# yuansliu/minicom

Measured on AMD Instinct MI355X. Metric: Mreads/s (sketch+index+overlap) on 150bp reads, 1/2/4/8 GPU; bit-exact decompress, higher is better.
Workload: dtype u64

## Files before the change

minicom_amd/csrc/api.hip:

```cpp
#include "mcom_dev.hpp"
#include "../../include/mcom_test.h"
#include <stdarg.h>
#include <stdlib.h>
#include <cxxabi.h>
#include <stdio.h>
#include <string.h>

int mcom_fail(mcom_ctx *ctx, int code, const char *fmt, ...)
{
	char buf[512];
	va_list ap;
	va_start(ap, fmt);
	vsnprintf(buf, sizeof buf, fmt, ap);
	va_end(ap);
	if (ctx) { ctx->err = buf; ctx->pin_wait.clear(); ctx->pin_off = 0; }
	return code;
}

#define MCOM_PIN_BYTES 4096
hipError_t mcom_d2h_async(mcom_ctx *ctx, void *dst, const void *src, size_t bytes)
{
	for (uint32_t q = 0; q < 8; ++q) {
		const mcom_ctx::ScanTotal &t = ctx->scan_last[(ctx->scan_last_at + 7u - q) % 8u];
		if (t.last && t.last == src && t.bytes == bytes && t.gen == ctx->launch_gen) { mcom_ctx::PinWait w{dst, 0, bytes}; w.from = ctx->scan_tot + t.slot; ctx->pin_wait.push_back(w); return hipSuccess; }
// ... 287 lines not shown
{
	if (!ctx || !name) return 0;
	if (!strcmp(name, "sort_overflow_segments")) return ctx->sort_overflow_segments;
	if (!strcmp(name, "sketch_strings")) return ctx->sketch_strings;
	return 0;
}
extern "C" int mcom_set_segment_capacity(mcom_ctx *ctx, uint32_t records)
{
	if (!ctx || records > 4096) return MCOM_E_ARG;
	ctx->seg_cap = records;
	return MCOM_OK;
}
extern "C" int mcom_set_consensus_capacity(mcom_ctx *ctx, uint32_t members)
{
	if (!ctx) return MCOM_E_ARG;
	ctx->bs_cap = members;
	return MCOM_OK;
}
extern "C" int mcom_set_sketch_kernel(mcom_ctx *ctx, int wave_per_string)
{
	if (!ctx) return MCOM_E_ARG;
	ctx->sketch_wave_only = wave_per_string == 1;
	ctx->sketch_ring64 = wave_per_string == 2;
	ctx->sketch_ring32_only = wave_per_string == 3;
	ctx->sketch_lane_always = wave_per_string >= 2;
	return MCOM_OK;
}
extern "C" int mcom_set_sketch_prefix_bits(mcom_ctx *ctx, int bits)
{
	if (!ctx || bits < 1 || bits > 30) return MCOM_E_ARG;
	ctx->sketch_prefix_bits = bits;
	return MCOM_OK;
}
extern "C" int mcom_set_claim_route(mcom_ctx *ctx, int route)
{
	if (!ctx || route < 0 || route > 3) return MCOM_E_ARG;
	ctx->claim_route = route;
	return MCOM_OK;
}
extern "C" int mcom_claim_fallbacks(const mcom_ctx *ctx) { return ctx ? (int)ctx->claim_fallbacks : 0; }
extern "C" int mcom_set_screen_route(mcom_ctx *ctx, int route)
{
	if (!ctx || route < 0 || route > 2) return MCOM_E_ARG;
	ctx->screen_route = route;
	return MCOM_OK;
}
extern "C" int mcom_screen_fallbacks(const mcom_ctx *ctx) { return ctx ? (int)ctx->screen_fallbacks : 0; }
extern "C" int mcom_set_lookup_route(mcom_ctx *ctx, int route)
{
	if (!ctx || route < 0 || route > 1) return MCOM_E_ARG;
	ctx->lookup_route = route;
	return MCOM_OK;
}
extern "C" int mcom_set_index_capacity(mcom_ctx *ctx, int entries)
{
	if (!ctx) return MCOM_E_ARG;
	ctx->cix_cap_set = entries >= 0; ctx->cix_cap = entries >= 0 ? (uint32_t)entries : 0u;
	return MCOM_OK;
}
```

minicom_amd/csrc/consensus_bs.hip:

```cpp
#include "mcom_dev.hpp"

#define BS_K 5
#define BS_NMAX 31u
#define BS_KM 7
#define BS_EVEN 0x5555555555555555ull

namespace {
template <int K> struct BsCnt { uint64_t p[K], q[K]; };

template <int K> __device__ __forceinline__ void bs_add(BsCnt<K> &c, uint64_t P, uint64_t Q)
{
#pragma unroll
	for (int b = 0; b < K; ++b) { uint64_t t = c.p[b] & P; c.p[b] ^= P; P = t; t = c.q[b] & Q; c.q[b] ^= Q; Q = t; }
}
template <int K> __device__ __forceinline__ void bs_sub(BsCnt<K> &c, uint64_t P, uint64_t Q)
{
#pragma unroll
	for (int b = 0; b < K; ++b) { uint64_t t = ~c.p[b] & P; c.p[b] ^= P; P = t; t = ~c.q[b] & Q; c.q[b] ^= Q; Q = t; }
}
template <int K> __device__ __forceinline__ void bs_best(const BsCnt<K> &c, uint64_t &lo, uint64_t &hi, uint64_t &nz)
{
	uint64_t best[K], cand[K];
#pragma unroll
	for (int b = 0; b < K; ++b) best[b] = c.p[b] & BS_EVEN;
	lo = 0; hi = 0;
	auto challenge = [&](int code) {
		uint64_t gt = 0, eq = BS_EVEN;
#pragma unroll
		for (int b = K - 1; b >= 0; --b) { gt |= eq & cand[b] & ~best[b]; eq &= ~(cand[b] ^ best[b]); }
#pragma unroll
		for (int b = 0; b < K; ++b) best[b] = (cand[b] & gt) | (best[b] & ~gt);
		lo = (code & 1) ? (lo | gt) : (lo & ~gt);
		hi = (code & 2) ? (hi | gt) : (hi & ~gt);
	};
#pragma unroll
	for (int b = 0; b < K; ++b) cand[b] = (c.p[b] >> 1) & BS_EVEN;
	challenge(1);
#pragma unroll
	for (int b = 0; b < K; ++b) cand[b] = c.q[b] & BS_EVEN;
	challenge(2);
#pragma unroll
	for (int b = 0; b < K; ++b) cand[b] = (c.q[b] >> 1) & BS_EVEN;
	challenge(3);
	nz = 0;
#pragma unroll
	for (int b = 0; b < K; ++b) nz |= best[b];
}
__device__ __forceinline__ uint64_t bs_rev(uint64_t x)
{
	x = __brevll(x);
	return ((x >> 1) & BS_EVEN) | ((x & BS_EVEN) << 1);
}
__device__ __forceinline__ uint64_t bs_span(int a, int b)
{
	if (b <= a) return 0;
	const uint64_t mb = b >= 32 ? ~0ull : ((1ull << (2 * b)) - 1), ma = (1ull << (2 * a)) - 1;
	return BS_EVEN & mb & ~ma;
}

#define BS_ORDER_GRID 1024
__global__ __launch_bounds__(256) void k_bs_sizes(const uint32_t *__restrict__ goff, uint32_t ng, uint32_t *__restrict__ bins)
{
	__shared__ uint32_t h[33];
	if (threadIdx.x < 33) h[threadIdx.x] = 0;
	__syncthreads();
	const uint32_t chunks = (ng + 255u) / 256u, per = (chunks + gridDim.x - 1) / gridDim.x;
	const uint32_t c0 = blockIdx.x * per, c1 = c0 + per < chunks ? c0 + per : chunks;
	for (uint32_t c = c0; c < c1; ++c) {
		const uint32_t g = c * 256u + threadIdx.x;
		if (g < ng) { const uint32_t n = goff[g + 1] - goff[g]; atomicAdd(&h[n < 32u ? n : 32u], 1u); }
	}
	__syncthreads();
	if (threadIdx.x < 33 && h[threadIdx.x]) atomicAdd(&bins[threadIdx.x], h[threadIdx.x]);
}
__global__ __launch_bounds__(256) void k_bs_order(const uint32_t *__restrict__ goff, uint32_t ng, const uint32_t *__restrict__ bins,
                                                  uint32_t *__restrict__ cursor, uint32_t *__restrict__ perm)
{
	__shared__ uint32_t h[33], base[33];
	if (threadIdx.x < 33) h[threadIdx.x] = 0;
	__syncthreads();
	const uint32_t chunks = (ng + 255u) / 256u, per = (chunks + gridDim.x - 1) / gridDim.x;
	const uint32_t c0 = blockIdx.x * per, c1 = c0 + per < chunks ? c0 + per : chunks;
	for (uint32_t c = c0; c < c1; ++c) {
		const uint32_t g = c * 256u + threadIdx.x;
		if (g < ng) { const uint32_t n = goff[g + 1] - goff[g]; atomicAdd(&h[n < 32u ? n : 32u], 1u); }
	}
	__syncthreads();
	if (threadIdx.x < 33) {
		const uint32_t b = threadIdx.x;
		uint32_t start = 0;
		if (b == 32) { for (uint32_t q = 0; q < 32; ++q) start += bins[q]; }
		else for (uint32_t q = b + 1; q < 32; ++q) start += bins[q];
		base[b] = start + (h[b] ? atomicAdd(&cursor[b], h[b]) : 0u);
		h[b] = 0;
	}
	__syncthreads();
	for (uint32_t c = c0; c < c1; ++c) {
		const uint32_t g = c * 256u + threadIdx.x;
		if (g < ng) { const uint32_t n = goff[g + 1] - goff[g], bin = n < 32u ? n : 32u; perm[base[bin] + atomicAdd(&h[bin], 1u)] = g; }
	}
}

__global__ __launch_bounds__(64) void k_group_consensus_bs(const uint64_t *__restrict__ packed, int W, uint64_t *__restrict__ members,
                                                           const uint32_t *__restrict__ goff, const uint32_t *__restrict__ perm, uint32_t nsmall,
                                                           int L, int k_orig, int e, int LG, int GPW,
                                                           uint8_t *__restrict__ keep, uint32_t *__restrict__ nkept,
                                                           uint16_t *__restrict__ svout, uint16_t *__restrict__ reflen,
                                                           uint8_t *__restrict__ refs, int ref_stride)
{
	__shared__ uint32_t S[2][64];
	__shared__ uint32_t M[64];
	__shared__ uint64_t CODE[64 + 64];
	const int lane = threadIdx.x;
	const int gs = lane / LG, u = lane - gs * LG;
	const uint32_t idx = blockIdx.x * (uint32_t)GPW + (uint32_t)gs;
	const bool valid = gs < GPW && idx < nsmall;
	const int TL = 2 * L;
	const uint32_t g = valid ? perm[idx] : 0u;
	const uint32_t m0 = valid ? goff[g] : 0u;
	const uint32_t n = valid ? goff[g + 1] - m0 : 0u;
	uint32_t nmax = n;
#pragma unroll
	for (int d = 32; d >= 1; d >>= 1) { const uint32_t o = (uint32_t)__shfl_xor((int)nmax, d, 64); nmax = o > nmax ? o : nmax; }
	S[0][lane] = 0; S[1][lane] = 0;
	const int col0 = 32 * u;
	int pos0 = 0;
	if (n) { const uint64_t y = members[m0]; int pos = (int)((uint32_t)y >> 1); if (y & 1) pos = L - pos + k_orig - 2; pos0 = pos; }
	struct Fetch { uint64_t y, wa, wb; int off, s0, sh; bool covered; };
	auto fetch_y = [&](uint32_t i) -> uint64_t { return i < n ? members[m0 + i] : 0ull; };
	auto fetch_rows = [&](uint32_t i, uint64_t y) -> Fetch {
		Fetch f; f.y = y;
		const uint32_t dir = (uint32_t)(y & 1);
		int pos = (int)((uint32_t)y >> 1);
		if (dir) pos = L - pos + k_orig - 2;
		f.off = pos0 - pos;
		f.s0 = col0 - f.off;
		f.covered = i < n && f.s0 < L && f.s0 + 32 > 0;
		const int t0 = dir ? L - 32 - f.s0 : f.s0;
		const int wj = t0 >> 5;
		f.sh = 2 * (t0 & 31);
		const uint64_t *row = packed + (size_t)(y >> 32) * W;
		f.wa = (f.covered && wj >= 0 && wj < W) ? row[wj] : 0ull;
		f.wb = (f.covered && f.sh && wj + 1 >= 0 && wj + 1 < W) ? row[wj + 1] : 0ull;
		return f;
	};
	auto finish = [&](const Fetch &f, uint64_t &x, uint64_t &cov) {
		x = f.sh ? (f.wa >> f.sh) | (f.wb << (64 - f.sh)) : f.wa;
		if (f.y & 1) x = ~bs_rev(x);
		cov = f.covered ? bs_span(f.s0 < 0 ? -f.s0 : 0, L - f.s0 < 32 ? L - f.s0 : 32) : 0ull;
	};
	auto planes = [&](uint64_t x, uint64_t cov, uint64_t &P, uint64_t &Q) {
		const uint64_t lo = x & BS_EVEN, hi = (x >> 1) & BS_EVEN;
		const uint64_t nh = cov & ~hi, hh = cov & hi;
		P = (nh & ~lo) | ((nh & lo) << 1);
		Q = (hh & ~lo) | ((hh & lo) << 1);
	};
	BsCnt<BS_K> c;
#pragma unroll
	for (int b = 0; b < BS_K; ++b) { c.p[b] = 0; c.q[b] = 0; }
	{
		uint64_t yn = fetch_y(0);
		Fetch cur = fetch_rows(0, yn);
		yn = fetch_y(1);
		for (uint32_t i = 0; i < nmax; ++i) {
			const Fetch nxt = fetch_rows(i + 1, yn);
			yn = fetch_y(i + 2);
			uint64_t x, cov, P, Q;
			finish(cur, x, cov);
			planes(x, cov, P, Q);
			bs_add(c, P, Q);
			cur = nxt;
		}
	}
	uint64_t rlo, rhi, nz;
	bs_best(c, rlo, rhi, nz);
	if (u == 0) M[gs] = (uint32_t)TL;
	__syncthreads();
	{
		const uint64_t empty = ~nz & BS_EVEN;
		if (valid && empty) { const int cnd = col0 + (__ffsll((unsigned long long)empty) - 1) / 2; if (cnd < TL) atomicMin(&M[gs], (uint32_t)cnd); }
	}
	__syncthreads();
	const int ref_len = (int)M[gs];
	const uint64_t inref = bs_span(0, ref_len - col0 < 0 ? 0 : (ref_len - col0 > 32 ? 32 : ref_len - col0));
	uint32_t nk = 0; int rend = 0;
	uint64_t yn = fetch_y(0);
	Fetch cur = fetch_rows(0, yn);
	yn = fetch_y(1);
	for (uint32_t i = 0; i < nmax; ++i) {
		const Fetch nxt = fetch_rows(i + 1, yn);
		yn = fetch_y(i + 2);
		uint64_t x, cov, P, Q;
		finish(cur, x, cov);
		const uint64_t y = cur.y; const int off = cur.off;
		const uint64_t lo = x & BS_EVEN, hi = (x >> 1) & BS_EVEN;
		const uint64_t mis = cov & (((lo ^ rlo) | (hi ^ rhi)) | ~inref);
		const uint32_t slot = i & 1u;
		if (mis) atomicAdd(&S[slot][gs], (uint32_t)__popcll(mis));
		__builtin_amdgcn_wave_barrier();
		const uint32_t dif = ((volatile uint32_t*)S[slot])[gs];
		__builtin_amdgcn_wave_barrier();
		if (u == 0) ((volatile uint32_t*)S[slot ^ 1u])[gs] = 0;
		const bool act = i < n;
		const bool kp = (int)dif <= e;
		if (act && kp) { ++nk; if (off + L > rend) rend = off + L; }
		if (__ballot(act && !kp)) {
			planes(x, (act && !kp) ? cov : 0ull, P, Q);
			bs_sub(c, P, Q);
		}
		if (act && u == 0) { keep[m0 + i] = kp ? 1 : 0; members[m0 + i] = (y >> 32 << 32) | ((uint64_t)off << 1) | (y & 1); }
		cur = nxt;
	}
	bs_best(c, rlo, rhi, nz);
	__syncthreads();
	if (u == 0) M[gs] = (uint32_t)ref_len;
	CODE[gs * (LG + 1) + u] = rlo | (rhi << 1);
	if (u == 0) CODE[gs * (LG + 1) + LG] = 0;
	__syncthreads();
	{
		const uint64_t first = nz & inref;
		if (valid && nk && first) atomicMin(&M[gs], (uint32_t)(col0 + (__ffsll((unsigned long long)first) - 1) / 2));
	}
	__syncthreads();
	const int sv = nk ? (int)M[gs] : 0;
	if (valid && nk) {
		uint8_t *out = refs + (size_t)g * ref_stride;
		const uint32_t *w32 = (const uint32_t*)&CODE[gs * (LG + 1)];
		const int n_out = rend - sv;
		for (int d = u; 4 * d < n_out; d += LG) {
			const int bit = 2 * (sv + 4 * d), wi = bit >> 5, sh = bit & 31;
			uint32_t v = w32[wi] >> sh;
			if (sh > 24) v |= w32[wi + 1] << (32 - sh);
			uint32_t ascii = 0;
#pragma unroll
			for (int r = 0; r < 4; ++r) ascii |= ((0x54474341u >> (8 * ((v >> (2 * r)) & 3u))) & 0xFFu) << (8 * r);
			if (4 * d + 4 <= n_out) *(uint32_t*)(out + 4 * d) = ascii;
			else for (int r = 0; 4 * d + r < n_out; ++r) out[4 * d + r] = (uint8_t)(ascii >> (8 * r));
		}
	}
	if (valid && u == 0) { nkept[g] = nk; svout[g] = (uint16_t)sv; reflen[g] = (uint16_t)(nk ? rend - sv : 0); }
}

__global__ __launch_bounds__(64) void k_merge_consensus_bs(const uint64_t *__restrict__ packed, int W, const uint64_t *__restrict__ members,
                                                           const uint64_t *__restrict__ joff, const uint64_t *__restrict__ roff,
                                                           const uint32_t *__restrict__ ujob, const uint32_t *__restrict__ uoff, uint32_t n_units, int L,
                                                           uint8_t *__restrict__ refs, const uint32_t *__restrict__ reg_lo, const uint32_t *__restrict__ reg_hi,
                                                           const uint32_t *__restrict__ toff, unsigned int *__restrict__ tflag, uint32_t *__restrict__ tlist,
                                                           unsigned int *__restrict__ tcount, uint32_t depth_cap)
{
	const uint32_t q = blockIdx.x * 64u + threadIdx.x;
	const bool valid = q < n_units;
	const uint32_t j = valid ? ujob[q] : 0u;
	long lo = 0, hi = 0, c0 = 0;
	uint64_t m0 = 0, m1 = 0;
	if (valid) {
		hi = reg_hi ? (long)reg_hi[j] : (long)(roff[j + 1] - roff[j]);
		lo = reg_lo ? (long)reg_lo[j] : 0;
		c0 = lo + 32l * (long)(q - uoff[j]);
		m0 = joff[j]; m1 = joff[j + 1];
	}
	const long ce = c0 + 32 < hi ? c0 + 32 : hi;
	uint64_t a = m0, b = m1;
	while (a < b) { const uint64_t mid = (a + b) >> 1; if ((long)((uint32_t)members[mid] >> 1) + L <= c0) a = mid + 1; else b = mid; }
	BsCnt<BS_KM> c;
// ... 30 lines not shown
				const int sh = 2 * (t0 & 31);
				uint64_t x = sh ? (wa >> sh) | (wb << (64 - sh)) : wa;
				if (dir) x = ~bs_rev(x);
				const int e0 = L - s0 < (int)(ce - c0) ? L - s0 : (int)(ce - c0);
				const uint64_t cov = bs_span(s0 < 0 ? -s0 : 0, e0);
				const uint64_t xl = x & BS_EVEN, xh = (x >> 1) & BS_EVEN;
				const uint64_t nh = cov & ~xh, hh = cov & xh;
				bs_add(c, (nh & ~xl) | ((nh & xl) << 1), (hh & ~xl) | ((hh & xl) << 1));
				++n;
			}
			++i;
			y = y1; wa = wa1; wb = wb1; y1 = y2;
		}
	}
	if (!valid) return;
	if (over) {
		const uint32_t t = toff[j] + (uint32_t)((c0 - lo) >> 9);
		if (atomicExch(&tflag[t], 1u) == 0u) tlist[atomicAdd(tcount, 1u)] = t;
		return;
	}
	uint64_t rlo, rhi, nz;
	bs_best(c, rlo, rhi, nz);
	const uint64_t code = rlo | (rhi << 1);
	uint8_t *out = refs + roff[j] + c0;
	const int cnt = (int)(ce - c0);
#pragma unroll
	for (int d = 0; d < 8; ++d) {
		if (4 * d >= cnt) break;
		const uint32_t v = (uint32_t)(code >> (8 * d)) & 0xFFu;
		uint32_t ascii = 0;
#pragma unroll
		for (int r = 0; r < 4; ++r) ascii |= ((0x54474341u >> (8 * ((v >> (2 * r)) & 3u))) & 0xFFu) << (8 * r);
		if (4 * d + 4 <= cnt) __builtin_memcpy(out + 4 * d, &ascii, 4);
		else for (int r = 0; 4 * d + r < cnt; ++r) out[4 * d + r] = (uint8_t)(ascii >> (8 * r));
	}
}
}

int mcom_group_consensus_small(mcom_ctx *ctx, const uint64_t *d_packed, uint64_t *d_members, const uint32_t *d_group_off, uint32_t n_groups,
                               int L, int k_orig, int e, uint8_t *d_keep, uint32_t *d_nkept, uint16_t *d_sv, uint16_t *d_reflen, uint8_t *d_refs,
                               int ref_stride, uint32_t **d_perm_out, uint32_t *n_small)
{
	*d_perm_out = nullptr; *n_small = 0;
	uint32_t *perm = nullptr;
	if (mcom_dmalloc(&perm, ((size_t)n_groups + 128) * 4) != hipSuccess) return mcom_fail(ctx, MCOM_E_NOMEM, "group order");
	uint32_t *bins = (uint32_t*)mcom_zeroed(ctx, perm + n_groups, 80 * 4), *cursor = bins ? bins + 40 : nullptr;
	hipError_t er = bins ? hipSuccess : hipErrorUnknown;
	const unsigned blocks = std::min<unsigned>((n_groups + 255) / 256, BS_ORDER_GRID);
	if (er == hipSuccess) {
		MCOM_LAUNCH(k_bs_sizes, dim3(blocks), dim3(256), 0, ctx->stream, d_group_off, n_groups, bins);
		MCOM_LAUNCH(k_bs_order, dim3(blocks), dim3(256), 0, ctx->stream, d_group_off, n_groups, bins, cursor, perm);
		er = hipGetLastError();
	}
	uint32_t nbig = 0;
	if (er == hipSuccess) er = mcom_d2h_async(ctx, &nbig, bins + 32, 4);
	if (er == hipSuccess) er = mcom_stream_sync(ctx);
	if (er != hipSuccess) { mcom_dfree(perm); return mcom_fail(ctx, MCOM_E_HIP, "group order: %s", hipGetErrorString(er)); }
	const uint32_t nsmall = n_groups - nbig;
	const int LG = (2 * L + 31) / 32, GPW = 64 / LG;
	if (nsmall) {
		McomProfScope ps_(ctx, PROF_CONSENSUS);
		MCOM_LAUNCH(k_group_consensus_bs, dim3((nsmall + GPW - 1) / GPW), dim3(64), 0, ctx->stream, d_packed, mcom_words_per_read(L), d_members, d_group_off, perm,
		                   nsmall, L, k_orig, e, LG, GPW, d_keep, d_nkept, d_sv, d_reflen, d_refs, ref_stride);
	}
	er = hipGetLastError();
	if (er != hipSuccess) { mcom_dfree(perm); return mcom_fail(ctx, MCOM_E_HIP, "group consensus: %s", hipGetErrorString(er)); }
	*d_perm_out = perm; *n_small = nsmall;
	return MCOM_OK;
}

int mcom_merge_consensus_units(mcom_ctx *ctx, const uint64_t *d_packed, const uint64_t *d_members, const uint64_t *d_job_off, const uint64_t *d_ref_off,
                               const uint32_t *d_ujob, const uint32_t *d_uoff, uint32_t n_units, int L, uint8_t *d_refs,
                               const uint32_t *d_reg_lo, const uint32_t *d_reg_hi, const uint32_t *d_toff, uint32_t n_tiles,
                               unsigned int *d_tflag, uint32_t *d_tlist, uint32_t *h_nlist)
{
	*h_nlist = 0;
	if (n_units == 0) return MCOM_OK;
	unsigned int *tcount = d_tflag + n_tiles;
	MCOM_HIP(ctx, hipMemsetAsync(d_tflag, 0, ((size_t)n_tiles + 1) * 4, ctx->stream));
	{
		McomProfScope ps_(ctx, PROF_CONSENSUS);
		MCOM_LAUNCH(k_merge_consensus_bs, dim3((n_units + 63) / 64), dim3(64), 0, ctx->stream, d_packed, mcom_words_per_read(L), d_members, d_job_off, d_ref_off,
		                   d_ujob, d_uoff, n_units, L, d_refs, d_reg_lo, d_reg_hi, d_toff, d_tflag, d_tlist, tcount,
		                   ctx->bs_cap && ctx->bs_cap < (1u << BS_KM) ? ctx->bs_cap : (1u << BS_KM) - 1u);
	}
	MCOM_LAUNCH_CHECK(ctx);
	MCOM_HIP(ctx, mcom_d2h_async(ctx, h_nlist, tcount, 4));
	MCOM_HIP(ctx, mcom_stream_sync(ctx));
	return MCOM_OK;
}
```

minicom_amd/csrc/mcom_dev.hpp:

```cpp
#pragma once
#include <hip/hip_runtime.h>
#include <stdint.h>
#include <stddef.h>
#include <map>
#include <string>
#include <vector>
#include "../../include/mcom.h"

enum McomProfId { PROF_CLASSIFY_PACK = 0, PROF_SKETCH_READS, PROF_RADIX_PASS, PROF_SKETCH_CONTIGS, PROF_FIND_NEXT,
                  PROF_DICT_BUILD, PROF_REALIGN_WINDOWS, PROF_CONSENSUS, PROF_CINDEX_BUILD, PROF_REALIGN_READS, PROF_COUNT };
struct McomProfSpan { int id; hipEvent_t a, b; };

struct mcom_ctx {
	int device;
	hipStream_t stream;
	std::string err;
	void *ws; size_t ws_bytes;
	int n_cu;
	bool prof_on = false;
	std::vector<McomProfSpan> prof_open;
	double prof_ms[PROF_COUNT] = {0};
	uint64_t prof_calls[PROF_COUNT] = {0};
	int prof_cur = PROF_COUNT;
	std::map<std::pair<int, const void *>, uint64_t> prof_kernels;
	uint32_t seg_cap = 0; uint64_t sort_overflow_segments = 0;
	uint64_t sketch_strings = 0;
	bool cix_cap_set = false; uint32_t cix_cap = 0;
	uint32_t bs_cap = 0;
	bool sketch_wave_only = false;
	bool sketch_lane_always = false;
	bool sketch_ring64 = false, sketch_ring32_only = false; int sketch_prefix_bits = 14;
	unsigned long long *scan_parts = nullptr; uint32_t scan_epoch = 0; volatile unsigned int *poison = nullptr; unsigned int *d_poison = nullptr;
	enum { SCAN_TOTALS = 64 };
	unsigned long long *scan_tot = nullptr, *d_scan_tot = nullptr;
	struct ScanTotal { const void *last; uint32_t bytes, slot, gen; } scan_last[8] = {}; uint32_t scan_last_at = 0, launch_gen = 1;
	int claim_route = 0; uint64_t claim_fallbacks = 0;
	unsigned int *screen_flag = nullptr;
	std::vector<void*> free_later;
	int screen_route = 0; uint64_t screen_fallbacks = 0;
	int lookup_route = 0;
	int verify_hash_bits = 64;
	struct ScreenArgs { const uint64_t *sgbits; size_t n_sg; int L, ininumdict, maxsearch, n_shares, share; } screen_args = {};
	enum { ZPOOL_BYTES = 64 * 1024 };
	unsigned char *zpool = nullptr; size_t zpool_used = 0; int zpool_half = 0;
	struct PinWait { void *dst; size_t off, bytes; const void *from = nullptr; };
	unsigned char *pin = nullptr; size_t pin_off = 0;
	std::vector<PinWait> pin_wait;
};

hipEvent_t mcom_prof_event_get();
void mcom_prof_event_put(hipEvent_t e);
struct McomProfScope {
	mcom_ctx *ctx; int idx;
	McomProfScope(mcom_ctx *c, int id) : ctx(c), idx(-1) {
		if (!c->prof_on) return;
		McomProfSpan s; s.id = id;
		if (!(s.a = mcom_prof_event_get())) return;
		if (!(s.b = mcom_prof_event_get())) { mcom_prof_event_put(s.a); return; }
		(void)hipEventRecord(s.a, c->stream);
		c->prof_open.push_back(s); idx = (int)c->prof_open.size() - 1;
		prev = c->prof_cur; c->prof_cur = id;
	}
	~McomProfScope() { if (idx >= 0) { (void)hipEventRecord(ctx->prof_open[idx].b, ctx->stream); ctx->prof_cur = prev; } }
	int prev = PROF_COUNT;
};
#define MCOM_LAUNCH(kernel, grid, block, lds, stream, ...) do { \
	++ctx->launch_gen; \
	if (ctx->prof_on) ++ctx->prof_kernels[std::make_pair(ctx->prof_cur, (const void*)&kernel)]; \
	hipLaunchKernelGGL(kernel, grid, block, lds, stream, __VA_ARGS__); } while (0)

int mcom_fail(mcom_ctx *ctx, int code, const char *fmt, ...);
hipError_t mcom_d2h_async(mcom_ctx *ctx, void *dst, const void *src, size_t bytes);
hipError_t mcom_stream_sync(mcom_ctx *ctx);
hipError_t mcom_stream_sync_poison(mcom_ctx *ctx, bool *poisoned);
int mcom_ws_reserve(mcom_ctx *ctx, size_t bytes);
void *mcom_zeroed(mcom_ctx *ctx, void *fallback, size_t bytes);
void mcom_ring_flush_slot(mcom_ctx *ctx, uint32_t slot);
unsigned long long *mcom_ring_slot(mcom_ctx *ctx, uint32_t *slot);
void mcom_ring_register(mcom_ctx *ctx, const void *d_result, uint32_t bytes, uint32_t slot);
hipError_t mcom_dmalloc(void **out, size_t bytes);
void mcom_dfree(void *p);
void mcom_dfree_later(mcom_ctx *ctx, void *p);
template <class T> static inline hipError_t mcom_dmalloc(T **out, size_t bytes) { return mcom_dmalloc((void**)out, bytes); }

int mcom_scan_u32(mcom_ctx *ctx, const uint32_t *in, uint32_t *out, size_t n, uint32_t *scratch);
size_t mcom_scan_scratch_elems(size_t n);
int mcom_scan_prepare(mcom_ctx *ctx);
size_t mcom_sort_ws_bytes(size_t n);
int mcom_sort_by_x(mcom_ctx *ctx, mcom_mm128 *d_a, size_t n, int bits, void *ws);
int mcom_sort_by_low_bits(mcom_ctx *ctx, mcom_mm128 *d_a, size_t n, int bits, void *ws);
int mcom_sort_by_low_bits_into_ws(mcom_ctx *ctx, const mcom_mm128 *d_src, mcom_mm128 *d_a, size_t n, int bits, void *ws, mcom_mm128 **d_sorted);
#define MCOM_GROUP_TILE 1280
#define MCOM_GROUP_SCRATCH(n) (4 * ((size_t)(n) / MCOM_GROUP_TILE + 1) + 16)
// ... 133 lines not shown
```

minicom_amd/hip.py:

```python
from __future__ import annotations

import ctypes as C
import os
import re

import numpy as np

HERE = os.path.dirname(os.path.abspath(__file__))
MM_DTYPE = np.dtype([("x", "<u8"), ("y", "<u8")])


class McomError(RuntimeError):
    pass


class DecodeSrc(C.Structure):
    _fields_ = [("d_text", C.c_void_p), ("text_bytes", C.c_uint64), ("d_line_start", C.c_void_p), ("verbatim", C.c_int),
                ("d_ref", C.c_void_p), ("ref_bytes", C.c_uint64), ("ref_const", C.c_int),
                ("d_cid", C.c_void_p), ("d_pos", C.c_void_p), ("d_coff", C.c_void_p), ("n_contigs", C.c_uint64),
                ("d_dir", C.c_void_p), ("dir_bytes", C.c_uint64)]


DECODE_F_BOUNDS, DECODE_F_LINE, DECODE_F_DUP, DECODE_F_DEST = 1, 2, 4, 8

# ... 131 lines not shown
    L.mcom_decode_pe_dest.restype = i32; L.mcom_decode_pe_dest.argtypes = [vp, vp, u64, u64, u64, vp, u64, u64, u64, vp, C.POINTER(u64), vp]
    L.mcom_decode_check_lines.restype = i32; L.mcom_decode_check_lines.argtypes = [vp, vp, u64, vp, u64, i32, i32, vp]
    L.mcom_decode_reads.restype = i32; L.mcom_decode_reads.argtypes = [vp, C.POINTER(DecodeSrc), u64, i32, vp, u64, vp, u64, vp, vp]
    L.mcom_verify_room.restype = u64; L.mcom_verify_room.argtypes = [u64, u64]
    L.mcom_verify_ordered.restype = i32; L.mcom_verify_ordered.argtypes = [vp, C.POINTER(VerifyTable), C.POINTER(VerifyTable), i32, C.POINTER(VerifyReport)]
    L.mcom_verify_multiset.restype = i32; L.mcom_verify_multiset.argtypes = [vp, C.POINTER(VerifyTable), C.POINTER(VerifyTable), i32, C.POINTER(VerifyReport)]
    L.mcom_set_verify_hash_bits.restype = i32; L.mcom_set_verify_hash_bits.argtypes = [vp, i32]
    L.mcom_rans_bound.restype = u64; L.mcom_rans_bound.argtypes = [u64]
    L.mcom_rans_encode.restype = i32; L.mcom_rans_encode.argtypes = [vp, vp, u64, vp, u64, C.POINTER(u64), i32]
    L.mcom_rans_decode.restype = i32; L.mcom_rans_decode.argtypes = [vp, vp, u64, vp, u64, C.POINTER(u64)]
    L.mcom_fastq_quality_rows.restype = i32; L.mcom_fastq_quality_rows.argtypes = [vp, vp, u64, vp, u64, u64, C.c_uint32, vp, u64, vp]
    L.mcom_fastq_emit.restype = i32; L.mcom_fastq_emit.argtypes = [vp, vp, u64, vp, u64, u64, u64, C.c_uint32, vp, C.POINTER(u64)]
    L.mcom_qual_bound.restype = u64; L.mcom_qual_bound.argtypes = [u64, C.c_uint32]
    L.mcom_qual_encode.restype = i32; L.mcom_qual_encode.argtypes = [vp, vp, u64, C.c_uint32, u64, vp, u64, C.POINTER(u64), i32]
    L.mcom_qual_gather_rows.restype = i32; L.mcom_qual_gather_rows.argtypes = [vp, vp, u64, C.c_uint32, u64, vp, u64, vp, u64, vp]
    L.mcom_dump_read_order.restype = i32; L.mcom_dump_read_order.argtypes = [vp, vp, u64, vp, u64, C.c_uint32, vp, C.POINTER(u64)]
    L.mcom_verify_multiset_parts.restype = i32; L.mcom_verify_multiset_parts.argtypes = [vp, C.POINTER(VerifyParts), C.POINTER(VerifyParts), i32, C.POINTER(VerifyReport)]
    L.mcom_qual_info.restype = i32; L.mcom_qual_info.argtypes = [vp, u64, C.POINTER(u64), C.POINTER(C.c_uint32)]
    L.mcom_qual_decode.restype = i32; L.mcom_qual_decode.argtypes = [vp, vp, u64, vp, u64, u64, C.POINTER(u64), C.POINTER(C.c_uint32)]
    L.mcom_name_bound.restype = u64; L.mcom_name_bound.argtypes = [u64]
    L.mcom_name_encode.restype = i32; L.mcom_name_encode.argtypes = [vp, vp, u64, u64, vp, u64, C.POINTER(u64), C.POINTER(u64)]
    L.mcom_name_info.restype = i32; L.mcom_name_info.argtypes = [vp, u64, C.POINTER(u64), C.POINTER(u64)]
    L.mcom_name_decode.restype = i32; L.mcom_name_decode.argtypes = [vp, vp, u64, vp, u64, C.POINTER(u64), C.POINTER(u64), vp]
    L.mcom_name_text_offsets.restype = i32; L.mcom_name_text_offsets.argtypes = [vp, vp, u64, u64, vp]
    L.mcom_name_compare.restype = i32; L.mcom_name_compare.argtypes = [vp, vp, vp, u64, vp, vp, u64, u64, C.POINTER(u64), C.POINTER(u64)]
    L.mcom_fastq_name_text.restype = i32; L.mcom_fastq_name_text.argtypes = [vp, vp, u64, vp, u64, u64, vp, u64, C.POINTER(u64), vp, vp]
    L.mcom_fastq_emit_named.restype = i32; L.mcom_fastq_emit_named.argtypes = [vp, vp, u64, vp, u64, vp, u64, vp, u64, C.c_uint32, vp, C.POINTER(u64)]
    L.mcom_bwt_bound.restype = u64; L.mcom_bwt_bound.argtypes = [u64]
    L.mcom_bwt_encode.restype = i32; L.mcom_bwt_encode.argtypes = [vp, vp, u64, vp, u64, C.POINTER(u64)]
    L.mcom_bwt_decode.restype = i32; L.mcom_bwt_decode.argtypes = [vp, vp, u64, vp, u64, C.POINTER(u64)]
    L.mcom_synth_reads.restype = i32
    L.mcom_synth_reads.argtypes = [vp, u64, u64, i32, i32, C.c_double, u64, u64, vp, sz]
    L.mcom_synth_reads_genome.restype = i32
    L.mcom_synth_reads_genome.argtypes = [vp, u64, u64, i32, i32, C.c_double, i32, u64, u64, vp, sz]
    _lib = L
    return L


def words_per_read(L: int) -> int:
    return (2 * L + 63) // 64


def _torch():
    import torch
    return torch


class Context:

    def __init__(self, device: int = 0, stream=None):
        torch = _torch()
        if not torch.cuda.is_available():
            raise McomError("no GPU visible: the minicom_amd product path has no CPU fallback")
        self.lib = load_library()
        self.device = torch.device("cuda", device)
        torch.cuda.set_device(self.device)
        self._stream = stream if stream is not None else torch.cuda.current_stream(self.device)
        h = C.c_void_p()
        rc = self.lib.mcom_create(C.byref(h), device, C.c_void_p(self._stream.cuda_stream))
        if rc:
            raise McomError(f"mcom_create failed ({rc})")
        self._h = h

    def close(self):
        if getattr(self, "_h", None):
            self.lib.mcom_destroy(self._h)
            self._h = None

    def __del__(self):
        try:
            self.close()
        except Exception:
            pass

    def _check(self, rc: int):
        if rc:
            raise McomError(f"mcom error {rc}: {self.lib.mcom_last_error(self._h).decode()}")

    def _p(self, t, dtype=None):
        if t is None:
            return C.c_void_p(0)
        assert t.is_cuda and t.is_contiguous(), "device, contiguous tensors only"
        if dtype is not None:
            assert t.dtype == dtype, (t.dtype, dtype)
        return C.c_void_p(t.data_ptr())

    def sync(self):
        self._check(self.lib.mcom_sync(self._h))

    def empty_records(self, n: int):
        torch = _torch()
        return torch.empty((n, 2), dtype=torch.int64, device=self.device)

    def process_reads(self, ascii_, L: int, k: int, e: int = 4, rid0: int = 0, want_nmask: bool = False):
        torch = _torch()
        n, pitch = ascii_.shape
        W = words_per_read(L)
        packed = torch.empty((n, W), dtype=torch.int64, device=self.device)
        cls = torch.empty(n, dtype=torch.uint8, device=self.device)
        ncnt = torch.empty(n, dtype=torch.int16, device=self.device)
        nmask = torch.empty((n, (L + 63) // 64), dtype=torch.int64, device=self.device) if want_nmask else None
        rec = self.empty_records(n)
        self._check(self.lib.mcom_process_reads(self._h, self._p(ascii_, torch.uint8), pitch, n, L, k, e, rid0,
                                                self._p(packed), self._p(cls), self._p(ncnt), self._p(nmask), self._p(rec)))
        return {"packed": packed, "cls": cls, "ncnt": ncnt, "nmask": nmask, "rec": rec}

# ... 20 lines not shown
        return out[: min(c, cap)], c

    def sketch_reads(self, packed, L: int, k: int, rids=None, rid0: int = 0, out=None):
        torch = _torch()
        n = int(rids.shape[0]) if rids is not None else int(packed.shape[0])
        rec = out if out is not None else self.empty_records(n)
        self._check(self.lib.mcom_sketch_reads(self._h, self._p(packed, torch.int64),
                                               self._p(rids, torch.int32) if rids is not None else C.c_void_p(0),
                                               n, L, k, rid0, self._p(rec)))
        return rec

    def hash64(self, kmers, k: int):
        torch = _torch()
        out = torch.empty_like(kmers)
        self._check(self.lib.mcom_hash64_batch(self._h, self._p(kmers, torch.int64), int(kmers.shape[0]), k, self._p(out)))
        return out

    def encode_byte(self, rows, cg, contig, pos, dirs, L: int):
        torch = _torch()
        n = int(rows.shape[0])
        ok = torch.empty(max(n, 1), dtype=torch.uint8, device=self.device)
        self._check(self.lib.mcom_encode_byte(self._h, self._p(rows, torch.int64), self._p(cg["cbits"]), self._p(cg["coff"]), self._p(contig, torch.int32),
                                              self._p(pos, torch.int32), self._p(dirs, torch.uint8), n, L, self._p(ok)))
        return ok[:n]

    def radix_sort_128x(self, rec):
        torch = _torch()
        self._check(self.lib.mcom_radix_sort_128x(self._h, self._p(rec, torch.int64), int(rec.shape[0])))
        return rec

    def counter(self, name: str) -> int:
        self.lib.mcom_counter.restype = C.c_uint64; self.lib.mcom_counter.argtypes = [C.c_void_p, C.c_char_p]
        return int(self.lib.mcom_counter(self._h, name.encode()))

    def set_segment_capacity(self, records: int):
        self.lib.mcom_set_segment_capacity.restype = C.c_int; self.lib.mcom_set_segment_capacity.argtypes = [C.c_void_p, C.c_uint32]
        self._check(self.lib.mcom_set_segment_capacity(self._h, records))

    def set_index_capacity(self, entries: int):
        self.lib.mcom_set_index_capacity.restype = C.c_int; self.lib.mcom_set_index_capacity.argtypes = [C.c_void_p, C.c_int]
        self._check(self.lib.mcom_set_index_capacity(self._h, entries))

    def set_sketch_kernel(self, wave_per_string):
        self.lib.mcom_set_sketch_kernel.restype = C.c_int; self.lib.mcom_set_sketch_kernel.argtypes = [C.c_void_p, C.c_int]
        self._check(self.lib.mcom_set_sketch_kernel(self._h, int(wave_per_string)))

    def set_sketch_prefix_bits(self, bits: int):
        self.lib.mcom_set_sketch_prefix_bits.restype = C.c_int; self.lib.mcom_set_sketch_prefix_bits.argtypes = [C.c_void_p, C.c_int]
        self._check(self.lib.mcom_set_sketch_prefix_bits(self._h, bits))

    def set_claim_route(self, route: int):
        self.lib.mcom_set_claim_route.restype = C.c_int; self.lib.mcom_set_claim_route.argtypes = [C.c_void_p, C.c_int]
        self._check(self.lib.mcom_set_claim_route(self._h, route))

    def claim_fallbacks(self) -> int:
        self.lib.mcom_claim_fallbacks.restype = C.c_int; self.lib.mcom_claim_fallbacks.argtypes = [C.c_void_p]
        return int(self.lib.mcom_claim_fallbacks(self._h))

    def set_screen_route(self, route: int):
        self.lib.mcom_set_screen_route.restype = C.c_int; self.lib.mcom_set_screen_route.argtypes = [C.c_void_p, C.c_int]
        self._check(self.lib.mcom_set_screen_route(self._h, route))

    def screen_fallbacks(self) -> int:
        self.lib.mcom_screen_fallbacks.restype = C.c_int; self.lib.mcom_screen_fallbacks.argtypes = [C.c_void_p]
        return int(self.lib.mcom_screen_fallbacks(self._h))

    def set_consensus_capacity(self, members: int):
        self.lib.mcom_set_consensus_capacity.restype = C.c_int; self.lib.mcom_set_consensus_capacity.argtypes = [C.c_void_p, C.c_uint32]
        self._check(self.lib.mcom_set_consensus_capacity(self._h, members))

    def sort_group(self, rec, L: int, k_orig: int, kmer: int, b: int = 14):
        torch = _torch()
        n = int(rec.shape[0])
        srt = self.empty_records(n)
        singles = torch.empty(max(n, 1), dtype=torch.int32, device=self.device)
        sord = torch.empty(max(n, 1), dtype=torch.int32, device=self.device)
        members = torch.empty(max(n, 1), dtype=torch.int64, device=self.device)
        goff = torch.empty(n // 2 + 2, dtype=torch.int32, device=self.device)
        cnt = (C.c_uint64 * 4)()
        self._check(self.lib.mcom_sort_group(self._h, self._p(rec, torch.int64), n, L, k_orig, kmer, b, self._p(srt),
                                             self._p(singles), self._p(sord), self._p(members), self._p(goff), cnt))
        nv, ns, ng, nm = (int(x) for x in cnt)
        return {"sorted": srt, "n_valid": nv, "singles": singles[:ns], "single_ord": sord[:ns], "members": members[:nm], "group_off": goff[:ng + 1] if n else goff[:0],
                "n_groups": ng}

    def upload_contigs(self, refs):
        torch = _torch()
        lens = np.array([len(r) for r in refs], dtype=np.int64)
        off = np.concatenate([[0], np.cumsum(lens)]).astype(np.int64)
        words = (2 * lens + 63) // 64 + 1
        coff = np.concatenate([[0], np.cumsum(words)[:-1]]).astype(np.int64) if len(refs) else np.zeros(0, np.int64)
        total = int(words.sum())
        seq = torch.from_numpy(np.frombuffer(b"".join(refs) + b"\0", dtype=np.uint8).copy()).to(self.device)
        d_off = torch.from_numpy(off).to(self.device)
        d_coff = torch.from_numpy(coff).to(self.device)
        d_clen = torch.from_numpy(lens.astype(np.int32)).to(self.device)
        cbits = torch.zeros(total + 1, dtype=torch.int64, device=self.device)
        self._check(self.lib.mcom_pack_contigs(self._h, self._p(seq), self._p(d_off), self._p(d_coff), len(refs), total, self._p(cbits)))
        return {"seq": seq, "off": d_off, "coff": d_coff, "clen": d_clen, "cbits": cbits, "n": len(refs), "lens": lens}

    def unpack_contigs(self, cbits, coff, off, n: int, byte_lo: int, byte_hi: int, seq):
        self.lib.mcom_unpack_contigs.restype = C.c_int
        self.lib.mcom_unpack_contigs.argtypes = [C.c_void_p] * 4 + [C.c_uint32, C.c_uint64, C.c_uint64, C.c_void_p]
        self._check(self.lib.mcom_unpack_contigs(self._h, self._p(cbits), self._p(coff), self._p(off), n, byte_lo, byte_hi, self._p(seq)))

    def sketch_contigs(self, seq, off, n: int, w: int, k: int, max_per_contig: int = 0, ids=None):
# ... 897 lines not shown
```

Before: 555.0.

## Specialize group consensus kernel by group size with cached member descriptors

Splits small groups into three size classes using the order histogram. Each class launches a templated consensus kernel whose bit-sliced counter width matches the class (K=3/4/5). Member positions and offsets are precomputed once into shared-memory descriptors, and row loads become branchless through clamped indices. The main loop is software-pipelined three members deep. For small and mid groups the shifted read words are cached in shared memory so the second pass can skip refetching them. The aim is to cut register pressure and redundant global loads in the consensus pass, at the cost of extra launches, dynamic shared memory, and a larger histogram copy back to the host.

```diff
diff --git a/minicom_amd/csrc/api.hip b/minicom_amd/csrc/api.hip
--- a/minicom_amd/csrc/api.hip
+++ b/minicom_amd/csrc/api.hip
@@ -363,6 +363,12 @@
 	ctx->lookup_route = route;
 	return MCOM_OK;
 }
+extern "C" int mcom_set_group_route(mcom_ctx *ctx, int route)
+{
+	if (!ctx || route < 0 || route > 1) return MCOM_E_ARG;
+	ctx->group_route = route;
+	return MCOM_OK;
+}
 extern "C" int mcom_set_index_capacity(mcom_ctx *ctx, int entries)
 {
 	if (!ctx) return MCOM_E_ARG;
diff --git a/minicom_amd/csrc/consensus_bs.hip b/minicom_amd/csrc/consensus_bs.hip
--- a/minicom_amd/csrc/consensus_bs.hip
+++ b/minicom_amd/csrc/consensus_bs.hip
@@ -1,9 +1,11 @@
 #include "mcom_dev.hpp"
 
-#define BS_K 5
 #define BS_NMAX 31u
 #define BS_KM 7
 #define BS_EVEN 0x5555555555555555ull
+#define BS_KEEPX_LO true
+#define BS_KEEPX_MID true
+#define BS_KEEPX_HI false
 
 namespace {
 template <int K> struct BsCnt { uint64_t p[K], q[K]; };
@@ -101,6 +103,7 @@
 	}
 }
 
+template <int K, int NCAP, bool KEEPX>
 __global__ __launch_bounds__(64) void k_group_consensus_bs(const uint64_t *__restrict__ packed, int W, uint64_t *__restrict__ members,
                                                            const uint32_t *__restrict__ goff, const uint32_t *__restrict__ perm, uint32_t nsmall,
                                                            int L, int k_orig, int e, int LG, int GPW,
@@ -108,9 +111,11 @@
                                                            uint16_t *__restrict__ svout, uint16_t *__restrict__ reflen,
                                                            uint8_t *__restrict__ refs, int ref_stride)
 {
+	static_assert(NCAP < (1 << K), "the counters must hold a full group");
 	__shared__ uint32_t S[2][64];
 	__shared__ uint32_t M[64];
 	__shared__ uint64_t CODE[64 + 64];
+	extern __shared__ uint64_t BS_DYN[];
 	const int lane = threadIdx.x;
 	const int gs = lane / LG, u = lane - gs * LG;
 	const uint32_t idx = blockIdx.x * (uint32_t)GPW + (uint32_t)gs;
@@ -124,30 +129,53 @@
 	for (int d = 32; d >= 1; d >>= 1) { const uint32_t o = (uint32_t)__shfl_xor((int)nmax, d, 64); nmax = o > nmax ? o : nmax; }
 	S[0][lane] = 0; S[1][lane] = 0;
 	const int col0 = 32 * u;
-	int pos0 = 0;
-	if (n) { const uint64_t y = members[m0]; int pos = (int)((uint32_t)y >> 1); if (y & 1) pos = L - pos + k_orig - 2; pos0 = pos; }
-	struct Fetch { uint64_t y, wa, wb; int off, s0, sh; bool covered; };
-	auto fetch_y = [&](uint32_t i) -> uint64_t { return i < n ? members[m0 + i] : 0ull; };
-	auto fetch_rows = [&](uint32_t i, uint64_t y) -> Fetch {
-		Fetch f; f.y = y;
-		const uint32_t dir = (uint32_t)(y & 1);
-		int pos = (int)((uint32_t)y >> 1);
-		if (dir) pos = L - pos + k_orig - 2;
-		f.off = pos0 - pos;
-		f.s0 = col0 - f.off;
+	uint64_t *DESC = BS_DYN + (valid ? gs * NCAP : 0);
+	uint64_t *X = BS_DYN + GPW * NCAP + lane;
+	{
+		int pos0 = 0;
+		if (n) { const uint64_t y = members[m0]; int pos = (int)((uint32_t)y >> 1); if (y & 1) pos = L - pos + k_orig - 2; pos0 = pos; }
+		for (uint32_t base = 0; base < nmax; base += 4u * (uint32_t)LG) {
+			uint64_t yy[4];
+#pragma unroll
+			for (int t = 0; t < 4; ++t) { const uint32_t i = base + (uint32_t)(u + t * LG); yy[t] = i < n ? members[m0 + i] : 0ull; }
+#pragma unroll
+			for (int t = 0; t < 4; ++t) {
+				const uint32_t i = base + (uint32_t)(u + t * LG);
+				const uint64_t y = yy[t];
+				int pos = (int)((uint32_t)y >> 1);
+				if (y & 1) pos = L - pos + k_orig - 2;
+				if (i < n) DESC[i] = (y & 0xFFFFFFFF00000000ull) | (uint32_t)(((pos0 - pos) << 1) | (int)(y & 1));
+			}
+		}
+	}
+	__syncthreads();
+	struct Fetch { uint64_t wa, wb; int s0, sh; uint32_t dir; bool covered; };
+	auto desc = [&](uint32_t i) -> uint64_t { return i < n ? DESC[i] : 0ull; };
+	auto desc_off = [](uint64_t d) -> int { return (int)(uint32_t)d >> 1; };
+	auto clampw = [&](int w) -> uint32_t { const int lo = w > 0 ? w : 0; return (uint32_t)(lo < W ? lo : W - 1); };
+	auto fetch_rows = [&](uint32_t i, uint64_t d) -> Fetch {
+		Fetch f;
+		f.dir = (uint32_t)(d & 1);
+		f.s0 = col0 - desc_off(d);
 		f.covered = i < n && f.s0 < L && f.s0 + 32 > 0;
-		const int t0 = dir ? L - 32 - f.s0 : f.s0;
+		const int t0 = f.dir ? L - 32 - f.s0 : f.s0;
 		const int wj = t0 >> 5;
 		f.sh = 2 * (t0 & 31);
-		const uint64_t *row = packed + (size_t)(y >> 32) * W;
-		f.wa = (f.covered && wj >= 0 && wj < W) ? row[wj] : 0ull;
-		f.wb = (f.covered && f.sh && wj + 1 >= 0 && wj + 1 < W) ? row[wj + 1] : 0ull;
+		const uint64_t row = (uint64_t)(f.covered ? (uint32_t)(d >> 32) : 0u) * (uint32_t)W;
+		f.wa = packed[row + clampw(wj)];
+		f.wb = packed[row + clampw(wj + 1)];
 		return f;
 	};
+	auto span_of = [&](bool covered, int s0) -> uint64_t {
+		const int a = s0 < 0 ? -s0 : 0, b = L - s0;
+		const uint64_t mb = b >= 32 ? ~0ull : ~(~0ull << (2 * (b & 31))), ma = ~0ull << (2 * (a & 31));
+		return covered ? BS_EVEN & mb & ma : 0ull;
+	};
 	auto finish = [&](const Fetch &f, uint64_t &x, uint64_t &cov) {
-		x = f.sh ? (f.wa >> f.sh) | (f.wb << (64 - f.sh)) : f.wa;
-		if (f.y & 1) x = ~bs_rev(x);
-		cov = f.covered ? bs_span(f.s0 < 0 ? -f.s0 : 0, L - f.s0 < 32 ? L - f.s0 : 32) : 0ull;
+		x = (f.wa >> f.sh) | ((f.wb << 1) << (63 - f.sh));
+		const uint64_t r = ~bs_rev(x);
+		x = f.dir ? r : x;
+		cov = span_of(f.covered, f.s0);
 	};
 	auto planes = [&](uint64_t x, uint64_t cov, uint64_t &P, uint64_t &Q) {
 		const uint64_t lo = x & BS_EVEN, hi = (x >> 1) & BS_EVEN;
@@ -155,23 +183,26 @@
 		P = (nh & ~lo) | ((nh & lo) << 1);
 		Q = (hh & ~lo) | ((hh & lo) << 1);
 	};
-	BsCnt<BS_K> c;
-#pragma unroll
-	for (int b = 0; b < BS_K; ++b) { c.p[b] = 0; c.q[b] = 0; }
-	{
-		uint64_t yn = fetch_y(0);
-		Fetch cur = fetch_rows(0, yn);
-		yn = fetch_y(1);
-		for (uint32_t i = 0; i < nmax; ++i) {
-			const Fetch nxt = fetch_rows(i + 1, yn);
-			yn = fetch_y(i + 2);
-			uint64_t x, cov, P, Q;
-			finish(cur, x, cov);
-			planes(x, cov, P, Q);
-			bs_add(c, P, Q);
-			cur = nxt;
-		}
-	}
+	auto for_members = [&](auto &&use) {
+		Fetch fa = fetch_rows(0, desc(0)), fb = fetch_rows(1, desc(1)), fc;
+		for (uint32_t i = 0; i < nmax; i += 3) {
+			fc = fetch_rows(i + 2, desc(i + 2)); use(i, fa);
+			if (i + 1 >= nmax) break;
+			fa = fetch_rows(i + 3, desc(i + 3)); use(i + 1, fb);
+			if (i + 2 >= nmax) break;
+			fb = fetch_rows(i + 4, desc(i + 4)); use(i + 2, fc);
+		}
+	};
+	BsCnt<K> c;
+#pragma unroll
+	for (int b = 0; b < K; ++b) { c.p[b] = 0; c.q[b] = 0; }
+	for_members([&](uint32_t i, const Fetch &f) {
+		uint64_t x, cov, P, Q;
+		finish(f, x, cov);
+		if (KEEPX) X[i * 64u] = x;
+		planes(x, cov, P, Q);
+		bs_add(c, P, Q);
+	});
 	uint64_t rlo, rhi, nz;
 	bs_best(c, rlo, rhi, nz);
 	if (u == 0) M[gs] = (uint32_t)TL;
@@ -184,15 +215,10 @@
 	const int ref_len = (int)M[gs];
 	const uint64_t inref = bs_span(0, ref_len - col0 < 0 ? 0 : (ref_len - col0 > 32 ? 32 : ref_len - col0));
 	uint32_t nk = 0; int rend = 0;
-	uint64_t yn = fetch_y(0);
-	Fetch cur = fetch_rows(0, yn);
-	yn = fetch_y(1);
-	for (uint32_t i = 0; i < nmax; ++i) {
-		const Fetch nxt = fetch_rows(i + 1, yn);
-		yn = fetch_y(i + 2);
-		uint64_t x, cov, P, Q;
-		finish(cur, x, cov);
-		const uint64_t y = cur.y; const int off = cur.off;
+	auto judge = [&](uint32_t i, uint64_t x, uint64_t cov) {
+		const bool act = i < n;
+		const uint64_t d = desc(i);
+		const int off = desc_off(d);
 		const uint64_t lo = x & BS_EVEN, hi = (x >> 1) & BS_EVEN;
 		const uint64_t mis = cov & (((lo ^ rlo) | (hi ^ rhi)) | ~inref);
 		const uint32_t slot = i & 1u;
@@ -201,15 +227,22 @@
 		const uint32_t dif = ((volatile uint32_t*)S[slot])[gs];
 		__builtin_amdgcn_wave_barrier();
 		if (u == 0) ((volatile uint32_t*)S[slot ^ 1u])[gs] = 0;
-		const bool act = i < n;
 		const bool kp = (int)dif <= e;
 		if (act && kp) { ++nk; if (off + L > rend) rend = off + L; }
 		if (__ballot(act && !kp)) {
+			uint64_t P, Q;
 			planes(x, (act && !kp) ? cov : 0ull, P, Q);
 			bs_sub(c, P, Q);
 		}
-		if (act && u == 0) { keep[m0 + i] = kp ? 1 : 0; members[m0 + i] = (y >> 32 << 32) | ((uint64_t)off << 1) | (y & 1); }
-		cur = nxt;
+		if (act && u == 0) { keep[m0 + i] = kp ? 1 : 0; members[m0 + i] = (d >> 32 << 32) | ((uint64_t)off << 1) | (d & 1); }
+	};
+	if (KEEPX) {
+		for (uint32_t i = 0; i < nmax; ++i) {
+			const int s0 = col0 - desc_off(desc(i));
+			judge(i, X[i * 64u], span_of(i < n && s0 < L && s0 + 32 > 0, s0));
+		}
+	} else {
+		for_members([&](uint32_t i, const Fetch &f) { uint64_t x, cov; finish(f, x, cov); judge(i, x, cov); });
 	}
 	bs_best(c, rlo, rhi, nz);
 	__syncthreads();
@@ -346,16 +379,26 @@
 		MCOM_LAUNCH(k_bs_order, dim3(blocks), dim3(256), 0, ctx->stream, d_group_off, n_groups, bins, cursor, perm);
 		er = hipGetLastError();
 	}
-	uint32_t nbig = 0;
-	if (er == hipSuccess) er = mcom_d2h_async(ctx, &nbig, bins + 32, 4);
+	uint32_t hb[33] = {0};
+	if (er == hipSuccess) er = mcom_d2h_async(ctx, hb, bins, sizeof hb);
 	if (er == hipSuccess) er = mcom_stream_sync(ctx);
 	if (er != hipSuccess) { mcom_dfree(perm); return mcom_fail(ctx, MCOM_E_HIP, "group order: %s", hipGetErrorString(er)); }
-	const uint32_t nsmall = n_groups - nbig;
+	const uint32_t nsmall = n_groups - hb[32];
 	const int LG = (2 * L + 31) / 32, GPW = 64 / LG;
 	if (nsmall) {
+		uint32_t n_hi = 0, n_mid = 0;
+		for (int q = 16; q < 32; ++q) n_hi += hb[q];
+		for (int q = 8; q < 16; ++q) n_mid += hb[q];
+		if (ctx->group_route == 1) { n_hi = nsmall; n_mid = 0; }
+		const uint32_t n_lo = nsmall - n_hi - n_mid;
 		McomProfScope ps_(ctx, PROF_CONSENSUS);
-		MCOM_LAUNCH(k_group_consensus_bs, dim3((nsmall + GPW - 1) / GPW), dim3(64), 0, ctx->stream, d_packed, mcom_words_per_read(L), d_members, d_group_off, perm,
-		                   nsmall, L, k_orig, e, LG, GPW, d_keep, d_nkept, d_sv, d_reflen, d_refs, ref_stride);
+#define MCOM_BS(K_, NCAP_, KEEPX_, first_, count_) if (count_) MCOM_LAUNCH((k_group_consensus_bs<K_, NCAP_, KEEPX_>), dim3(((count_) + GPW - 1) / GPW), dim3(64), \
+	((size_t)GPW * NCAP_ + ((KEEPX_) ? (size_t)NCAP_ * 64 : 0)) * 8, ctx->stream, d_packed, mcom_words_per_read(L), d_members, d_group_off, perm + (first_), \
+	(count_), L, k_orig, e, LG, GPW, d_keep, d_nkept, d_sv, d_reflen, d_refs, ref_stride)
+		MCOM_BS(5, 31, BS_KEEPX_HI, 0u, n_hi);
+		MCOM_BS(4, 15, BS_KEEPX_MID, n_hi, n_mid);
+		MCOM_BS(3, 7, BS_KEEPX_LO, n_hi + n_mid, n_lo);
+#undef MCOM_BS
 	}
 	er = hipGetLastError();
 	if (er != hipSuccess) { mcom_dfree(perm); return mcom_fail(ctx, MCOM_E_HIP, "group consensus: %s", hipGetErrorString(er)); }
diff --git a/minicom_amd/csrc/mcom_dev.hpp b/minicom_amd/csrc/mcom_dev.hpp
--- a/minicom_amd/csrc/mcom_dev.hpp
+++ b/minicom_amd/csrc/mcom_dev.hpp
@@ -39,6 +39,7 @@
 	std::vector<void*> free_later;
 	int screen_route = 0; uint64_t screen_fallbacks = 0;
 	int lookup_route = 0;
+	int group_route = 0;
 	int verify_hash_bits = 64;
 	struct ScreenArgs { const uint64_t *sgbits; size_t n_sg; int L, ininumdict, maxsearch, n_shares, share; } screen_args = {};
 	enum { ZPOOL_BYTES = 64 * 1024 };
diff --git a/minicom_amd/hip.py b/minicom_amd/hip.py
--- a/minicom_amd/hip.py
+++ b/minicom_amd/hip.py
@@ -207,6 +207,8 @@
         torch = _torch()
         if not torch.cuda.is_available():
             raise McomError("no GPU visible: the minicom_amd product path has no CPU fallback")
+        if not 0 <= int(device) < torch.cuda.device_count():
+            raise McomError("no GPU %d (%d visible)" % (int(device), torch.cuda.device_count()))
         self.lib = load_library()
         self.device = torch.device("cuda", device)
         torch.cuda.set_device(self.device)
@@ -333,6 +335,10 @@
     def set_claim_route(self, route: int):
         self.lib.mcom_set_claim_route.restype = C.c_int; self.lib.mcom_set_claim_route.argtypes = [C.c_void_p, C.c_int]
         self._check(self.lib.mcom_set_claim_route(self._h, route))
+
+    def set_group_route(self, route: int):
+        self.lib.mcom_set_group_route.restype = C.c_int; self.lib.mcom_set_group_route.argtypes = [C.c_void_p, C.c_int]
+        self._check(self.lib.mcom_set_group_route(self._h, route))
 
     def claim_fallbacks(self) -> int:
         self.lib.mcom_claim_fallbacks.restype = C.c_int; self.lib.mcom_claim_fallbacks.argtypes = [C.c_void_p]
```

Measured after the change: 559.0 (median of 6 runs). No clear change (+0.7%).
